# datavizweb/async-rl-tensorflow

Hardware: AMD Instinct MI355X
Metric: env-steps/sec (whole node), Pong-v0 84×84×4, 1/2/4/8 MI355X + CPU ref (higher is better)
Workload: dtype fp32; 1 GPU; Pong-v0, 256 envs batched per MI355X, n-step=5, A3C conv net (nips trunk); frames=M1: raw RGB 210x160x3 + screen, game=Pong-v0, trunk=nips, head=feed-forward, env=device, envs_per_gpu=256, n_step=5, action_size=6, algo=a3c, parallelism=dp1, hipgraph=False

## Files before the change

async-rl-tensorflow_amd/csrc/net_fwd.hip:

```cpp
#include <cstdlib>
#include "net.h"
#include "lstm.h"
#include "gemm.h"
#include "net_bwd.h"
#include "env_dev.h"
#include "screen_atari.h"
#include "net_head.h"

#define XB_BYTES (HIST * PLANE * 2)
#ifdef C2_FP32
#define L1S_BYTES (C1_P * L1S_LD * 4)
#else
#define L1T_LD 56
#define L1S_BYTES (C1_P * L1T_LD * 2)
#endif
#define CONV12_SMEM (XB_BYTES + L1S_BYTES)
#define CONV12_SMEM_U8 (HIST * PLANE + L1S_BYTES)

__device__ inline void split3_bits(float w, uint32_t& h, uint32_t& m, uint32_t& l) {
#pragma clang fp contract(off)
  h = bf16_rn_bits(w);
  const float r1 = w - __uint_as_float(h << 16);
  m = bf16_rn_bits(r1);
  const float r2 = r1 - __uint_as_float(m << 16);
// ... 233 lines not shown
      for (int t = 0; t < 3; ++t) bq[t] = bn[t];
    }
  }
#else
#pragma unroll
  for (int kh = 0; kh < C2_K; ++kh)
#pragma unroll
    for (int kw = 0; kw < C2_K; ++kw)
#pragma unroll
      for (int mi = 0; mi < 2; ++mi) {
        if (mi >= nm) break;
        f32x4 a = *(const f32x4*)(l1s + (pos0[mi] + kh * C1_O + kw) * L1S_LD + 4 * j4);
        f32x4& c = (kw & 1) ? acc2b[mi] : acc2[mi];
#pragma unroll
        for (int c4 = 0; c4 < 4; ++c4)
          c = __builtin_amdgcn_mfma_f32_16x16x4f32(a[c4], w2r[(kh * 4 + kw) * 4 + c4], c, 0, 0, 0);
      }
#endif
#pragma unroll
  for (int mi = 0; mi < 2; ++mi) acc2[mi] += acc2b[mi];
#pragma unroll
  for (int mi = 0; mi < 2; ++mi) {
    if (mi >= nm) break;
#pragma unroll
    for (int r = 0; r < 4; ++r) {
      const int q = 16 * (grp + 4 * mi) + 4 * j4 + r;
      const float v = fmaxf(acc2[mi][r] + bias2, 0.f);
      if (q < C2_Q) st_act(act_l2 + b * FLAT + q * C2_N + 16 * nt + i16, v);
      if (L2M && l2m) {
        const uint64_t bal = __ballot(v > 0.f);
        if (i16 == 0 && q < C2_Q)
          ((uint16_t*)l2m)[(b * C2_Q + q) * 2 + nt] = (uint16_t)(bal >> (16 * j4));
      }
    }
  }
}

static_assert(W1S_ELEMS * 2 <= L1S_BYTES, "conv1 weights staged in the l1 region");
template <bool SAVE_L1, bool EW, bool U8>
__device__ inline void conv12_core(const uint8_t* x8, const uint16_t* xb, float* l1s, int64_t b,
                                   const uint16_t* __restrict__ w1s, const float* __restrict__ b1,
                                   const float* __restrict__ W2, float* __restrict__ act_l1,
                                   float* __restrict__ act_l2, float (&w2r)[64], float bias2,
                                   uint64_t* dbg = nullptr, uint32_t* __restrict__ l2m = nullptr) {
  const int lane = threadIdx.x & 63;
  uint4* wl = (uint4*)l1s;
  for (int i = threadIdx.x; i < W1S_ELEMS / 8; i += blockDim.x) wl[i] = ((const uint4*)w1s)[i];
  __syncthreads();
  if (dbg && threadIdx.x == 0) dbg[11] = __builtin_readcyclecounter();
  f32x4 acc[C1_TILES];
#pragma unroll
  for (int i = 0; i < C1_TILES; ++i) acc[i] = (f32x4){0.f, 0.f, 0.f, 0.f};
  conv1_accum<U8, 0, HIST>(x8, xb, acc, [&](int f) { return __builtin_bit_cast(bf16x8, wl[f * 64 + lane]); });
  lds_only_barrier();
  conv12_finish<SAVE_L1, EW>(acc, l1s, b, w1s, b1, W2, act_l1, act_l2, w2r, bias2, dbg, l2m);
}


template <bool SAVE_L1, bool EW, bool U8>
__global__ void __launch_bounds__(512) k_conv12_fwd(StateAddr sa, int64_t B,
                                                    const uint16_t* __restrict__ w1s,
                                                    const float* __restrict__ b1,
                                                    const float* __restrict__ W2,
                                                    const float* __restrict__ b2,
                                                    float* __restrict__ act_l1,
                                                    float* __restrict__ act_l2,
                                                    uint32_t* __restrict__ l2m) {
  WGLOG(3);
  extern __shared__ __attribute__((aligned(16))) uint8_t smem[];
  uint16_t* xb = (uint16_t*)smem;
  uint8_t* x8 = smem;
  float* l1s = (float*)(smem + (U8 ? HIST * PLANE : XB_BYTES));
  const int64_t b = blockIdx.x;
  const int lane = threadIdx.x & 63, wid = threadIdx.x >> 6;
  const int i16 = lane & 15, j4 = lane >> 4;
  const int64_t tau0 = sa.tau_ptr ? *sa.tau_ptr : 0;
  WG_T0();

  constexpr int NCH = HIST * (PLANE / 16);
  constexpr int PER = (NCH + 511) / 512;
  auto stage_chunk = [&](int i, const uint4 v) {
    if constexpr (U8) {
      ((uint4*)x8)[i] = v;
      return;
    }
    const int c = i / (PLANE / 16), j = i - c * (PLANE / 16);
    const uint32_t w[4] = {v.x, v.y, v.z, v.w};
    uint32_t o[8];
#pragma unroll
    for (int q = 0; q < 4; ++q) {
      const float f0 = (float)(w[q] & 255u), f1 = (float)((w[q] >> 8) & 255u);
      const float f2 = (float)((w[q] >> 16) & 255u), f3 = (float)(w[q] >> 24);
      o[2 * q] = __builtin_amdgcn_perm(__float_as_uint(f1), __float_as_uint(f0), 0x07060302u);
      o[2 * q + 1] = __builtin_amdgcn_perm(__float_as_uint(f3), __float_as_uint(f2), 0x07060302u);
    }
    uint4* dst = (uint4*)(xb + c * PLANE + 16 * j);
    dst[0] = make_uint4(o[0], o[1], o[2], o[3]);
    dst[1] = make_uint4(o[4], o[5], o[6], o[7]);
  };
  auto chunk_src = [&](int i) -> uint4 {
    const int c = i / (PLANE / 16), j = i - c * (PLANE / 16);
    return ((const uint4*)state_plane(sa, b, c, tau0))[j];
  };
  uint4 sv[PER];
  if (EW) {
#pragma unroll
    for (int k = 0; k < PER; ++k) sv[k] = chunk_src(min((int)threadIdx.x + 512 * k, NCH - 1));
  } else {
    for (int i = threadIdx.x; i < NCH; i += 512) stage_chunk(i, chunk_src(i));
  }
  const int nt = wid & 1, grp = wid >> 1;
  float w2r[64];
#ifdef C2_FP32
  if (EW) {
#pragma unroll
    for (int kk = 0; kk < 16; ++kk)
#pragma unroll
      for (int c4 = 0; c4 < 4; ++c4) w2r[kk * 4 + c4] = W2[(kk * C1_N + 4 * j4 + c4) * C2_N + 16 * nt + i16];
  }
#endif
  const float bias2 = b2[16 * nt + i16];
  if (EW) {
#pragma unroll
    for (int k = 0; k < PER; ++k) {
      const int i = threadIdx.x + 512 * k;
      if (i < NCH) stage_chunk(i, sv[k]);
    }
  }

  conv12_core<SAVE_L1, EW, U8>(x8, xb, l1s, b, w1s, b1, W2, act_l1, act_l2, w2r, bias2, nullptr, l2m);
  WG_T1(act_l2 + b * FLAT);
}

template <int GAME = A3C_GAME_SYNTH>
__global__ void __launch_bounds__(256) k_head_fwd(const float* __restrict__ h3, int64_t B,
                                                  const float* __restrict__ Wp, const float* __restrict__ bp,
                                                  const float* __restrict__ Wv, const float* __restrict__ bv,
                                                  int A, int zs, float* __restrict__ z, HeadSelect sel) {
  WGLOG(4);
  __shared__ __attribute__((aligned(16))) f32x4 l3s[4][64];
  const int lane = threadIdx.x & 63;
  const int64_t b = (int64_t)blockIdx.x * 4 + (threadIdx.x >> 6);
  if (b >= B) return;
  float myz;
  if (sel.fc_part) {
    f32x4 fp[FC_NS];
#pragma unroll
    for (int w = 0; w < FC_NS; ++w) fp[w] = *(const f32x4*)(sel.fc_part + ((int64_t)w * B + b) * FC + 4 * lane);
    const f32x4 fb = *(const f32x4*)(sel.fc_bias + 4 * lane);
    f32x4 v = fp[0];
#pragma unroll
    for (int w = 1; w < FC_NS; ++w) v += fp[w];
#pragma unroll
    for (int c4 = 0; c4 < 4; ++c4) v[c4] = fmaxf(v[c4] + fb[c4], 0.f);
    l3s[threadIdx.x >> 6][lane] = v;
    if (sel.l3_out) *(f32x4*)(sel.l3_out + b * FC + 4 * lane) = v;
    myz = head_row((const float*)l3s[threadIdx.x >> 6], 0, Wp, bp, Wv, bv, A, lane);
  } else {
    myz = head_row(h3, b, Wp, bp, Wv, bv, A, lane);
  }
  if (lane < zs) z[b * zs + lane] = myz;
  if (sel.mode >= 0) (void)head_act<GAME>(myz, lane, A, sel, b);
  if (sel.adv_ptr && blockIdx.x == 0 && threadIdx.x == 0) *sel.adv_ptr += sel.adv_n;
}

template <int W = FC, bool PLAY = false, int GAME = A3C_GAME_SYNTH>
__device__ inline int32_t head_act_env(const float* __restrict__ h3, const float* __restrict__ Wp,
                                       const float* __restrict__ bp, const float* __restrict__ Wv,
                                       const float* __restrict__ bv, int A, int zs, float* __restrict__ z,
                                       const HeadSelect& sel, int64_t b, int64_t tau, uint64_t* dbg,
                                       const float* hrow = nullptr, const uint8_t* frozen = nullptr) {
  __shared__ int32_t s_act;
  __shared__ uint32_t s_draw, s_term;
  const int lane = threadIdx.x & 63, wid = threadIdx.x >> 6;
  const int e = (int)b;
  if constexpr (PLAY) {
    if (frozen[e]) return -1;
  }
  const int64_t nxt = ((tau + 1) & 1) * (int64_t)sel.par_E + e;
  if (wid == 0) {
    const float eps = sel_eps(sel, e, tau);
    u32x4 x;
    float myz;
    if constexpr (W == FC) {
      myz = hrow ? head_row(hrow, 0, Wp, bp, Wv, bv, A, lane, [&]() { x = action_draw(sel, b, tau); })
                 : head_row(h3, b, Wp, bp, Wv, bv, A, lane, [&]() { x = action_draw(sel, b, tau); });
    } else {
      auto mid = [&]() { x = action_draw(sel, b, tau); };
      myz = hrow ? head_row<decltype(mid), W>(hrow, 0, Wp, bp, Wv, bv, A, lane, mid)
                 : head_row<decltype(mid), W>(h3, b, Wp, bp, Wv, bv, A, lane, mid);
    }
    if (dbg) {
      if (lane == 0) dbg[1] = __builtin_readcyclecounter() + (uint64_t)(myz * 0.f);
    } else if (lane < zs) {
      z[b * zs + lane] = myz;
    }
    const int32_t a = select_with(myz, lane, A, sel.mode, x, eps);
    if (lane == 0) {
      sel.actions[b] = a;
      s_act = a;
      if (dbg) dbg[2] = __builtin_readcyclecounter() + (uint64_t)a * 0;
    }
  } else if (wid == 1 && lane == 0 && sel.env_on) {
    const int64_t cur = (tau & 1) * (int64_t)sel.par_E + e;
    const uint32_t id = (uint32_t)(sel.env_id_base + e);
    EnvState s = env_load(sel.envb, cur);
    uint32_t draw;
    if constexpr (GAME == A3C_GAME_CATCH) {
      draw = catch_act_pre(s, sel.envp.action_repeat);
    } else {
      draw = env_act_pre(s, sel.envp, id, !PLAY);
      if constexpr (!PLAY) sel.rewards[e] = fmaxf(-1.0f, fminf(1.0f, s.reward));
      if (sel.rewards_raw) sel.rewards_raw[e] = s.reward;
    }
    sel.terms[e] = (uint8_t)s.terminal;
    s_draw = draw;
    if constexpr (PLAY) {
      s_term = 0;
      env_store(sel.envb, nxt, s, false);
      env_store(sel.envb, cur, s, false);
    } else {
      s_term = s.terminal;
      if (s.terminal) {
        game_new_random_game<GAME>(s, sel.envp, id);
        env_store(sel.envb, nxt, s);
      } else {
        env_store(sel.envb, nxt, s, false);
      }
    }
    if (dbg) dbg[17] = __builtin_readcyclecounter();
  }
  __syncthreads();
  int32_t frame;
  if (sel.env_on) {
    float reward = 0.f;
    if constexpr (GAME == A3C_GAME_CATCH) {
      frame = catch_act_post(s_draw, (uint32_t)s_act, reward);
    } else {
      frame = env_frame_of(s_draw + sel.frame_salt, (uint32_t)s_act, sel.envp);
#ifdef A3C_ABL_FRAME
      frame = e & 63;
#endif
    }
    if (threadIdx.x == 0) {
      if constexpr (GAME == A3C_GAME_CATCH) {
        if constexpr (!PLAY) sel.rewards[e] = reward;
        if (sel.rewards_raw) sel.rewards_raw[e] = reward;
        if constexpr (PLAY) sel.envb.reward[nxt] = sel.envb.reward[(tau & 1) * (int64_t)sel.par_E + e] = reward;
      }
      sel.frames_out[e] = frame;
      if (!s_term) sel.envb.frame[nxt] = frame;
      if constexpr (PLAY) sel.envb.frame[(tau & 1) * (int64_t)sel.par_E + e] = frame;
    }
  } else {
    frame = sel.frames_out[b];
  }
  if (dbg && threadIdx.x == 0) dbg[3] = __builtin_readcyclecounter();
  return frame;
}

template <int HS_THREADS, int W = FC, int GAME = A3C_GAME_SYNTH>
__global__ void __launch_bounds__(HS_THREADS) k_head_screen(const float* __restrict__ h3,
                                                            const float* __restrict__ Wp,
                                                            const float* __restrict__ bp,
                                                            const float* __restrict__ Wv,
                                                            const float* __restrict__ bv, int A, int zs,
                                                            float* __restrict__ z, HeadSelect sel) {
  extern __shared__ __attribute__((aligned(16))) uint8_t smem[];
  const int64_t b = blockIdx.x;
  const int64_t tau = *sel.tau_ptr + sel.tau_add;
  WG_T0();
  uint64_t* dbg = nullptr;
#ifdef HS_TIMES
  dbg = blockIdx.x == HS_TIMES ? (uint64_t*)z : nullptr;
  if (dbg && threadIdx.x == 0) dbg[0] = __builtin_readcyclecounter();
#endif
  const int32_t frame = head_act_env<W, false, GAME>(h3, Wp, bp, Wv, bv, A, zs, z, sel, b, tau, dbg);
  uint8_t* slot = sel.ring + b * sel.R * PLANE + ((tau + 1) % sel.R) * PLANE;
  if (sel.frame84)
    atari::copy_frame84<HS_THREADS>(sel.pool + (int64_t)frame * PLANE, slot);
  else
    atari::screen_frame<HS_THREADS>(sel.pool + (int64_t)frame * (atari::IH * atari::IW * 3), slot, smem, dbg);
  WG_T1(z + b * zs);
}

template <int HS_THREADS, int W, int GAME = A3C_GAME_SYNTH>
__global__ void __launch_bounds__(HS_THREADS) k_head_screen_play(const float* __restrict__ h3,
                                                                 const float* __restrict__ Wp,
                                                                 const float* __restrict__ bp,
                                                                 const float* __restrict__ Wv,
                                                                 const float* __restrict__ bv, int A, int zs,
                                                                 float* __restrict__ z, HeadSelect sel,
                                                                 const uint8_t* __restrict__ frozen) {
  extern __shared__ __attribute__((aligned(16))) uint8_t smem[];
  const int64_t b = blockIdx.x;
  const int64_t tau = *sel.tau_ptr + sel.tau_add;
  const int32_t frame = head_act_env<W, true, GAME>(h3, Wp, bp, Wv, bv, A, zs, z, sel, b, tau, nullptr, nullptr, frozen);
  if (frame < 0) return;
  uint8_t* slot = sel.ring + b * sel.R * PLANE + ((tau + 1) % sel.R) * PLANE;
  if (sel.frame84)
    atari::copy_frame84<HS_THREADS>(sel.pool + (int64_t)frame * PLANE, slot);
  else
    atari::screen_frame<HS_THREADS>(sel.pool + (int64_t)frame * (atari::IH * atari::IW * 3), slot, smem, nullptr);
}

#define HSC_X8_OFF (((SCREEN_FRAME_SMEM_NOKV) + 15) / 16 * 16)
#define HSC_X8_BYTES ((HIST - 1) * 2 * 3 * 64 * 16)
#define HSC_SMEM (HSC_X8_OFF + HSC_X8_BYTES)
#define HSC_KV_OFF (PLANE * 2)
static_assert(L1S_BYTES <= SCREEN_FRAME_SMEM_NOKV, "l1 overlays the screen scratch");
static_assert(HSC_KV_OFF % 16 == 0 && HSC_KV_OFF + SCREEN_KV_BYTES <= HSC_X8_BYTES, "tap table in the x8 region");
static_assert(HSC_SMEM + 16 + 4096 <= 160 * 1024 - 82944, "rollout workgroup beside a compact conv backward one");
template <bool SAVE_L1, bool L2M, int GAME = A3C_GAME_SYNTH>
__global__ void __launch_bounds__(512) __attribute__((amdgpu_waves_per_eu(4))) k_head_screen_conv12(const float* __restrict__ h3,
                                                            const float* __restrict__ Wp,
                                                            const float* __restrict__ bp,
                                                            const float* __restrict__ Wv,
                                                            const float* __restrict__ bv, int A, int zs,
                                                            float* __restrict__ z, HeadSelect sel,
                                                            Conv12Next nx) {
  WGLOG(1);
  extern __shared__ __attribute__((aligned(16))) uint8_t smem[];
  uint8_t* x8 = smem + HSC_X8_OFF;
  const int64_t b = blockIdx.x;
  const int64_t tau = *sel.tau_ptr + sel.tau_add;
  const int64_t tau0 = *nx.sa.tau_ptr;
  WG_T0();
  unsigned long long* srec = span_rec(nx.sa, tau0);
  span_begin(srec);
  uint64_t* dbg = nullptr;
#ifdef HS_TIMES
  dbg = blockIdx.x == HS_TIMES ? (uint64_t*)z : nullptr;
  if (dbg && threadIdx.x == 0) dbg[0] = __builtin_readcyclecounter();
#endif
  constexpr int NCH3 = (HIST - 1) * (PLANE / 16);
  constexpr int PT = 512 - 128;
  constexpr int PER3 = (NCH3 + PT - 1) / PT;
  constexpr int NWF = (HIST - 1) * 2 * 3 * 64;
  constexpr int PERW = NWF / PT;
  static_assert(NWF % PT == 0 && NWF * 16 <= HSC_X8_BYTES, "old-plane conv1 weights in the x8 region");
  static_assert((HIST - 1) * PLANE * 2 <= 51 * 1024, "old planes as bf16 in the screen scratch");
  static_assert(PLANE * 2 <= HSC_X8_BYTES, "new plane as bf16 in the x8 region");
  const int fwid = threadIdx.x >> 6, flane = threadIdx.x & 63;
  const bool fold = sel.fc_part != nullptr;
  f32x4 fbias = {0.f, 0.f, 0.f, 0.f};
  f32x4 fpart[FC_NS];
  if (fold && fwid == 0) {
#pragma unroll
    for (int w = 0; w < FC_NS; ++w)
      fpart[w] = *(const f32x4*)(sel.fc_part + ((int64_t)w * gridDim.x + b) * FC + 4 * flane);
    fbias = *(const f32x4*)(sel.fc_bias + 4 * flane);
  }
  const int pt = (int)threadIdx.x - 128;
  uint4 pv[PER3];
  if (pt >= 0) {
#pragma unroll
    for (int k = 0; k < PER3; ++k) {
      const int i = min(pt + PT * k, NCH3 - 1);
      const int c = i / (PLANE / 16), j = i - c * (PLANE / 16);
      pv[k] = ((const uint4*)state_plane(nx.sa, b, c, tau0))[j];
    }
    const int wbase = (fwid - 2) * 64;
#pragma unroll
    for (int k = 0; k < PERW; ++k)
      glds16((const uint4*)nx.w1s + wbase + PT * k + flane, (uint4*)x8 + wbase + PT * k);
#ifdef HS_TIMES
    if (dbg && pt == 0) dbg[16] = __builtin_readcyclecounter() + (pv[0].x & 0);
#endif
  }
  const float* hrow = nullptr;
  if (fold) {
    f32x4* fl = (f32x4*)smem;
    if (fwid == 0) {
      f32x4 v = fpart[0];
#pragma unroll
      for (int w = 1; w < FC_NS; ++w) v += fpart[w];
#pragma unroll
      for (int c4 = 0; c4 < 4; ++c4) v[c4] = fmaxf(v[c4] + fbias[c4], 0.f);
      fl[flane] = v;
      *(f32x4*)(sel.l3_out + b * FC + 4 * flane) = v;
    }
    hrow = (const float*)fl;
  }
  const int32_t frame = head_act_env<FC, false, GAME>(h3, Wp, bp, Wv, bv, A, zs, z, sel, b, tau, dbg, hrow);
  uint16_t* xold = (uint16_t*)smem;
  uint4* wlds = (uint4*)x8;
  if (pt >= 0) {
    asm volatile("s_waitcnt vmcnt(0)" ::: "memory");
#pragma unroll
    for (int k = 0; k < PER3; ++k) {
      const int i = pt + PT * k;
      if (i < NCH3) {
        uint4* d = (uint4*)(xold + 16 * i);
        const uint2 a0 = atari::u8x4_to_bf16x4(pv[k].x), a1 = atari::u8x4_to_bf16x4(pv[k].y);
        const uint2 a2 = atari::u8x4_to_bf16x4(pv[k].z), a3 = atari::u8x4_to_bf16x4(pv[k].w);
        d[0] = make_uint4(a0.x, a0.y, a1.x, a1.y);
        d[1] = make_uint4(a2.x, a2.y, a3.x, a3.y);
      }
    }
  }
  const int lane = threadIdx.x & 63, wid = threadIdx.x >> 6;
  f32x4 acc[C1_TILES];
#pragma unroll
  for (int i = 0; i < C1_TILES; ++i) acc[i] = (f32x4){0.f, 0.f, 0.f, 0.f};
  auto conv1_old = [&]() {
    lds_only_barrier();
    conv1_accum<false, 0, HIST - 1, false>(nullptr, xold, acc,
                                           [&](int f) { return __builtin_bit_cast(bf16x8, wlds[f * 64 + lane]); });
    lds_only_barrier();
  };
  uint16_t* xnew = (uint16_t*)x8;
  uint8_t* slot = sel.ring + b * sel.R * PLANE + ((tau + 1) % sel.R) * PLANE;
  if (sel.frame84)
    atari::copy_frame84<512>(sel.pool + (int64_t)frame * PLANE, slot, xnew, conv1_old);
  else
    atari::screen_frame<512>(sel.pool + (int64_t)frame * (atari::IH * atari::IW * 3), slot, smem, dbg, xnew,
                             conv1_old, (int*)(x8 + HSC_KV_OFF));
  if (dbg && threadIdx.x == 0) dbg[9] = __builtin_readcyclecounter();
  uint4 wn[6];
#pragma unroll
  for (int f = 0; f < 6; ++f) wn[f] = ((const uint4*)nx.w1s)[((HIST - 1) * 6 + f) * 64 + lane];
  float w2r[64];
  const float bias2 = nx.b2[16 * (wid & 1) + (lane & 15)];
  __syncthreads();
  if (dbg && threadIdx.x == 0) dbg[11] = __builtin_readcyclecounter();
  conv1_accum<false, HIST - 1, HIST>(nullptr, xnew - (HIST - 1) * PLANE, acc, [&](int f) {
    return __builtin_bit_cast(bf16x8, wn[f - (HIST - 1) * 6]);
  });
  conv12_finish<SAVE_L1, false, L2M>(acc, (float*)smem, b, nx.w1s, nx.b1, nx.W2, SAVE_L1 ? nx.act_l1 : nullptr,
                                nx.act_l2, w2r, bias2, dbg, nx.l2m);
  span_end(srec);
  if (dbg) {
    __syncthreads();
    if (threadIdx.x == 0) dbg[10] = __builtin_readcyclecounter();
  }
  WG_T1(z + b * zs);
}

__global__ void __launch_bounds__(256) k_select(const float* __restrict__ z, int64_t B, int zs, int A,
                                                HeadSelect sel) {
  const int lane = threadIdx.x & 63;
  const int64_t b = (int64_t)blockIdx.x * 4 + (threadIdx.x >> 6);
  if (b >= B) return;
  float myz = lane < zs ? z[b * zs + lane] : 0.f;
  int32_t a = select_from_lanes(myz, lane, A, sel, b);
  if (lane == 0) sel.actions[b] = a;
}

int a3c_fc_fwd_launch(const float* A, const float* W, const float* bias, float* C, int64_t M, hipStream_t s,
                      const float* Wrows = nullptr);

template <int HS_THREADS, int W, int GAME = A3C_GAME_SYNTH>
__global__ void __launch_bounds__(HS_THREADS) k_head_screen_fold(const float* __restrict__ part, int nsplit,
                                                                 int64_t pstride, const float* __restrict__ fbias,
                                                                 float* __restrict__ hout,
                                                                 const float* __restrict__ Wp,
                                                                 const float* __restrict__ bp,
                                                                 const float* __restrict__ Wv,
                                                                 const float* __restrict__ bv, int A, int zs,
                                                                 float* __restrict__ z, HeadSelect sel) {
  extern __shared__ __attribute__((aligned(16))) uint8_t smem[];
  __shared__ __attribute__((aligned(16))) float hrow[W];
  const int64_t b = blockIdx.x;
  const int64_t tau = *sel.tau_ptr + sel.tau_add;
  for (int i = threadIdx.x; i < W; i += HS_THREADS) {
    const float v = fmaxf(sum_strided(part + b * W + i, nsplit, pstride) + fbias[i], 0.f);
    hrow[i] = v;
    hout[b * W + i] = v;
  }
  __syncthreads();
  const int32_t frame = head_act_env<W, false, GAME>(nullptr, Wp, bp, Wv, bv, A, zs, z, sel, b, tau, nullptr, hrow);
  uint8_t* slot = sel.ring + b * sel.R * PLANE + ((tau + 1) % sel.R) * PLANE;
  if (sel.frame84)
    atari::copy_frame84<HS_THREADS>(sel.pool + (int64_t)frame * PLANE, slot);
  else
    atari::screen_frame<HS_THREADS>(sel.pool + (int64_t)frame * (atari::IH * atari::IW * 3), slot, smem, nullptr);
}

static bool catch_on(const HeadSelect& sel) { return sel.env_on && sel.envp.game == A3C_GAME_CATCH; }
static int catch_fold_launch(const float* part, int nsplit, const float* fbias, float* l4, const float* Wp,
                             const float* bp, const float* Wv, const float* bv, int A, int zs, int64_t B, float* z,
                             const HeadSelect& sel, int nt, hipStream_t s);
static int catch_head_screen_launch(int W, const float* h, const float* Wp, const float* bp, const float* Wv,
                                    const float* bv, int A, int zs, int64_t B, float* z, const HeadSelect& sel, int nt,
                                    hipStream_t s);
static int catch_play_launch(int W, const float* h, const float* Wp, const float* bp, const float* Wv, const float* bv,
                             int A, int zs, int64_t B, float* z, const HeadSelect& sel, const uint8_t* frozen, int nt,
                             hipStream_t s);
static int catch_conv12_launch(const float* h, const float* Wp, const float* bp, const float* Wv, const float* bv, int A,
                               int zs, int64_t B, float* z, const HeadSelect& sel, const Conv12Next& nx, hipStream_t s);
static int catch_head_fwd_launch(const float* h, const float* Wp, const float* bp, const float* Wv, const float* bv, int A,
                                 int zs, int64_t B, float* z, const HeadSelect& sel, hipStream_t s);
static void catch_set_smem();

int a3c_head_screen_fold_launch(const float* part, int nsplit, const float* fbias, float* l4, const float* Wp,
                                const float* bp, const float* Wv, const float* bv, int A, int zs, int64_t B, float* z,
                                const HeadSelect& sel, hipStream_t s) {
  static const int env_t = (int)A3C_AB_KNOB("A3C_HS_THREADS", 0);
  const int nt = env_t ? env_t : (a3c_shared_gpu() ? 512 : 1024);
  const int64_t ps = B * 512;
  if (catch_on(sel)) return catch_fold_launch(part, nsplit, fbias, l4, Wp, bp, Wv, bv, A, zs, B, z, sel, nt, s);
  if (nt == 1024)
    hipLaunchKernelGGL((k_head_screen_fold<1024, 512>), dim3((unsigned)B), dim3(1024), SCREEN_FRAME_SMEM, s, part,
                       nsplit, ps, fbias, l4, Wp, bp, Wv, bv, A, zs, z, sel);
  else
    hipLaunchKernelGGL((k_head_screen_fold<512, 512>), dim3((unsigned)B), dim3(512), SCREEN_FRAME_SMEM, s, part,
                       nsplit, ps, fbias, l4, Wp, bp, Wv, bv, A, zs, z, sel);
  A3C_CHECK(hipGetLastError());
  return 0;
}

int a3c_head_screen_wide_launch(const float* l4, const float* Wp, const float* bp, const float* Wv, const float* bv,
                                int A, int zs, int64_t B, float* z, const HeadSelect& sel, hipStream_t s) {
  static const int env_t = (int)A3C_AB_KNOB("A3C_HS_THREADS", 0);
  const int nt = env_t ? env_t : (a3c_shared_gpu() ? 512 : 1024);
  if (catch_on(sel)) return catch_head_screen_launch(512, l4, Wp, bp, Wv, bv, A, zs, B, z, sel, nt, s);
  if (nt == 1024)
    hipLaunchKernelGGL((k_head_screen<1024, 512>), dim3((unsigned)B), dim3(1024), SCREEN_FRAME_SMEM, s, l4, Wp, bp,
                       Wv, bv, A, zs, z, sel);
  else
    hipLaunchKernelGGL((k_head_screen<512, 512>), dim3((unsigned)B), dim3(512), SCREEN_FRAME_SMEM, s, l4, Wp, bp, Wv,
                       bv, A, zs, z, sel);
  A3C_CHECK(hipGetLastError());
  return 0;
}

int a3c_head_screen_play_launch(int W, const float* h, const float* Wp, const float* bp, const float* Wv,
                                const float* bv, int A, int zs, int64_t B, float* z, const HeadSelect& sel,
                                const uint8_t* frozen, hipStream_t s) {
  if (B <= 0) return 0;
  if (!frozen || !sel.tau_ptr || !sel.env_on || !sel.ring || !sel.pool || !sel.rewards_raw || !sel.terms ||
      !sel.frames_out || !sel.actions || sel.mode < 0 || sel.par_E < B || (W != FC && W != 512))
    return a3c_set_error(A3C_ERR_INVALID, "a3c_head_screen_play", "bad argument");
  const int nt = a3c_shared_gpu() ? 512 : 1024;
  if (catch_on(sel)) return catch_play_launch(W, h, Wp, bp, Wv, bv, A, zs, B, z, sel, frozen, nt, s);
#define HSP_GO(T, WW) hipLaunchKernelGGL((k_head_screen_play<T, WW>), dim3((unsigned)B), dim3(T), SCREEN_FRAME_SMEM, s, h, \
                                         Wp, bp, Wv, bv, A, zs, z, sel, frozen)
  if (W == FC) {
    if (nt == 1024) HSP_GO(1024, FC);
    else HSP_GO(512, FC);
  } else {
    if (nt == 1024) HSP_GO(1024, 512);
    else HSP_GO(512, 512);
  }
#undef HSP_GO
  A3C_CHECK(hipGetLastError());
  return 0;
}

int a3c_head_screen_conv12_launch(const NetLayout& L, const float* P, const float* act_l3, int64_t B, float* z,
                                  const HeadSelect& sel, const Conv12Next& nx, hipStream_t s);
int a3c_forward_launch(const NetLayout& L, const float* params, const uint8_t* prep, const StateAddr& sa,
                       int64_t B, float* act_l1, float* act_l2, float* act_l3, float* z, const HeadSelect& sel,
                       hipStream_t s, const LstmStep* ls, bool skip_conv12, const Conv12Next* next,
                       float* fc_part, uint32_t* l2m, const uint8_t* play_frozen) {
  if (B <= 0) return 0;
  if (play_frozen && (next || fc_part || skip_conv12 || sel.mode < 0 || !sel.env_on || !sel.ring))
    return a3c_set_error(A3C_ERR_INVALID, "a3c_forward", "the play step runs unfused, with the device env and the fused screen");
  if (L.lstm != (ls != nullptr))
    return a3c_set_error(A3C_ERR_INVALID, "a3c_forward", "the LSTM head needs its recurrent state");
  const float* P = params;
  if (!skip_conv12) {
    int rc0 = a3c_conv12_launch(L, P, prep, sa, B, act_l1, act_l2, s, l2m);
    if (rc0) return rc0;
  }
  const bool part_lstm = fc_part && ls != nullptr;
  const bool part = fc_part && (part_lstm || (next ? sel.mode >= 0 && sel.env_on && sel.ring : sel.mode < 0));
  const bool fold_fc = part_lstm && ls->fc_tick;
  int rc = fold_fc ? a3c_fc_part_fold_launch(act_l2, (const float*)(prep + PREP_W1S_BYTES), fc_part, B, ls->fc_tick,
                                             P + L.off[T_FCB], act_l3, s)
         : part ? a3c_fc_part_launch(act_l2, (const float*)(prep + PREP_W1S_BYTES), fc_part, B, s)
                : a3c_fc_fwd_launch(act_l2, (const float*)(prep + PREP_W1S_BYTES), P + L.off[T_FCB], act_l3, B, s,
                                    P + L.off[T_FCW]);
  if (rc) return rc;
  const float* head_in = act_l3;
  if (ls) {
    LstmStep st = *ls;
    if (part_lstm && !fold_fc) {
      st.fc_part = fc_part;
      st.fc_bias = P + L.off[T_FCB];
      st.l3_out = act_l3;
    }
    rc = a3c_lstm_fwd_launch(P + L.off[T_LB], act_l3, st, B, s);
    if (rc) return rc;
    head_in = ls->h;
  }
  const float* Wv = L.algo == A3C_ALGO_A3C ? P + L.off[T_VW] : nullptr;
  const float* bv = L.algo == A3C_ALGO_A3C ? P + L.off[T_VB] : nullptr;
  if (sel.mode >= 0 && sel.env_on && sel.ring && next) {
    HeadSelect hs = sel;
    if (part && !part_lstm) {
      hs.fc_part = fc_part;
      hs.fc_bias = P + L.off[T_FCB];
      hs.l3_out = act_l3;
    }
    return a3c_head_screen_conv12_launch(L, P, head_in, B, z, hs, *next, s);
  }
  if (next) return a3c_set_error(A3C_ERR_INVALID, "a3c_forward", "conv fusion needs the fused env screen");
  if (play_frozen)
    return a3c_head_screen_play_launch(FC, head_in, P + L.off[T_HW], P + L.off[T_HB], Wv, bv, L.A, L.zs, B, z, sel,
                                       play_frozen, s);
  if (sel.mode >= 0 && sel.env_on && sel.ring)
    return a3c_head_screen_launch(L, P, head_in, B, z, sel, s);
  else {
    HeadSelect hs = sel;
    if (part && !part_lstm) {
      hs.fc_part = fc_part;
      hs.fc_bias = P + L.off[T_FCB];
      hs.l3_out = act_l3;
    }
    if (hs.mode >= 0 && catch_on(hs))
      return catch_head_fwd_launch(head_in, P + L.off[T_HW], P + L.off[T_HB], Wv, bv, L.A, L.zs, B, z, hs, s);
    hipLaunchKernelGGL(k_head_fwd<>, dim3((unsigned)((B + 3) / 4)), dim3(256), 0, s, head_in, B,
                       P + L.off[T_HW], P + L.off[T_HB], Wv, bv, L.A, L.zs, z, hs);
  }
  A3C_CHECK(hipGetLastError());
  return 0;
}

int a3c_head_screen_launch(const NetLayout& L, const float* P, const float* act_l3, int64_t B, float* z,
                           const HeadSelect& sel, hipStream_t s) {
  const float* Wv = L.algo == A3C_ALGO_A3C ? P + L.off[T_VW] : nullptr;
  const float* bv = L.algo == A3C_ALGO_A3C ? P + L.off[T_VB] : nullptr;
  static const int env_t = (int)A3C_AB_KNOB("A3C_HS_THREADS", 0);
  const int nt = env_t ? env_t : (a3c_shared_gpu() ? 512 : 1024);
  if (catch_on(sel))
    return catch_head_screen_launch(FC, act_l3, P + L.off[T_HW], P + L.off[T_HB], Wv, bv, L.A, L.zs, B, z, sel, nt, s);
  if (nt == 1024)
    hipLaunchKernelGGL(k_head_screen<1024>, dim3((unsigned)B), dim3(1024), SCREEN_FRAME_SMEM, s, act_l3,
                       P + L.off[T_HW], P + L.off[T_HB], Wv, bv, L.A, L.zs, z, sel);
  else
    hipLaunchKernelGGL(k_head_screen<512>, dim3((unsigned)B), dim3(512), SCREEN_FRAME_SMEM, s, act_l3,
                       P + L.off[T_HW], P + L.off[T_HB], Wv, bv, L.A, L.zs, z, sel);
  A3C_CHECK(hipGetLastError());
  return 0;
}

int a3c_head_screen_conv12_launch(const NetLayout& L, const float* P, const float* act_l3, int64_t B, float* z,
                                  const HeadSelect& sel, const Conv12Next& nx, hipStream_t s) {
  const float* Wv = L.algo == A3C_ALGO_A3C ? P + L.off[T_VW] : nullptr;
  const float* bv = L.algo == A3C_ALGO_A3C ? P + L.off[T_VB] : nullptr;
  if (!nx.sa.tau_ptr || !sel.tau_ptr)
    return a3c_set_error(A3C_ERR_INVALID, "a3c_head_screen_conv12", "device tau counters required");
  if (catch_on(sel))
    return catch_conv12_launch(act_l3, P + L.off[T_HW], P + L.off[T_HB], Wv, bv, L.A, L.zs, B, z, sel, nx, s);
#define HSC_GO(S, M) hipLaunchKernelGGL((k_head_screen_conv12<S, M>), dim3((unsigned)B), dim3(512), HSC_SMEM, s, act_l3, \
                                        P + L.off[T_HW], P + L.off[T_HB], Wv, bv, L.A, L.zs, z, sel, nx)
  if (nx.act_l1 && nx.l2m) HSC_GO(true, true);
  else if (nx.act_l1) HSC_GO(true, false);
  else if (nx.l2m) HSC_GO(false, true);
  else HSC_GO(false, false);
#undef HSC_GO
  A3C_CHECK(hipGetLastError());
  return 0;
}

int a3c_conv12_launch(const NetLayout& L, const float* P, const uint8_t* prep, const StateAddr& sa, int64_t B,
                      float* act_l1, float* act_l2, hipStream_t s, uint32_t* l2m) {
  if (!prep) return a3c_set_error(A3C_ERR_INVALID, "a3c_conv12_launch", "prepared forward weights missing");
  const uint16_t* w1s = (const uint16_t*)prep;
  const bool ew = !a3c_shared_gpu();
  static const int env_u8 = (int)A3C_AB_KNOB("A3C_C12_U8", -1);
  const bool u8 = env_u8 >= 0 ? env_u8 != 0 : !ew;
#define CONV12_ARGS sa, B, w1s, P + L.off[T_L1B], P + L.off[T_L2W], P + L.off[T_L2B], act_l1, act_l2, l2m
#define CONV12_GO(S, E, U) \
  hipLaunchKernelGGL((k_conv12_fwd<S, E, U>), dim3((unsigned)B), dim3(512), U ? CONV12_SMEM_U8 : CONV12_SMEM, s, CONV12_ARGS)
  if (u8) {
    if (act_l1 && ew) CONV12_GO(true, true, true);
    else if (act_l1) CONV12_GO(true, false, true);
    else if (ew) CONV12_GO(false, true, true);
    else CONV12_GO(false, false, true);
  } else {
    if (act_l1 && ew) CONV12_GO(true, true, false);
    else if (act_l1) CONV12_GO(true, false, false);
    else if (ew) CONV12_GO(false, true, false);
    else CONV12_GO(false, false, false);
  }
#undef CONV12_GO
#undef CONV12_ARGS
  A3C_CHECK(hipGetLastError());
  return 0;
}

int a3c_select_launch(const float* z, int64_t B, int zs, int A, const HeadSelect& sel, hipStream_t s) {
  if (B <= 0) return 0;
  hipLaunchKernelGGL(k_select, dim3((unsigned)((B + 3) / 4)), dim3(256), 0, s, z, B, zs, A, sel);
  A3C_CHECK(hipGetLastError());
  return 0;
}

void a3c_conv12_set_smem() {
#define C12_SMEM(S, E, U)                                                                        \
  (void)hipFuncSetAttribute((const void*)k_conv12_fwd<S, E, U>, hipFuncAttributeMaxDynamicSharedMemorySize, \
                            U ? CONV12_SMEM_U8 : CONV12_SMEM)
  C12_SMEM(true, true, false); C12_SMEM(true, false, false); C12_SMEM(false, true, false); C12_SMEM(false, false, false);
  C12_SMEM(true, true, true); C12_SMEM(true, false, true); C12_SMEM(false, true, true); C12_SMEM(false, false, true);
#undef C12_SMEM
  (void)hipFuncSetAttribute((const void*)k_head_screen_conv12<true, true>, hipFuncAttributeMaxDynamicSharedMemorySize,
                            HSC_SMEM);
  (void)hipFuncSetAttribute((const void*)k_head_screen_conv12<true, false>, hipFuncAttributeMaxDynamicSharedMemorySize,
                            HSC_SMEM);
  (void)hipFuncSetAttribute((const void*)k_head_screen_conv12<false, true>, hipFuncAttributeMaxDynamicSharedMemorySize,
                            HSC_SMEM);
  (void)hipFuncSetAttribute((const void*)k_head_screen_conv12<false, false>, hipFuncAttributeMaxDynamicSharedMemorySize,
                            HSC_SMEM);
  (void)hipFuncSetAttribute((const void*)k_head_screen<512>, hipFuncAttributeMaxDynamicSharedMemorySize,
                            SCREEN_FRAME_SMEM);
  (void)hipFuncSetAttribute((const void*)k_head_screen<1024>, hipFuncAttributeMaxDynamicSharedMemorySize,
                            SCREEN_FRAME_SMEM);
  (void)hipFuncSetAttribute((const void*)k_head_screen<512, 512>, hipFuncAttributeMaxDynamicSharedMemorySize,
                            SCREEN_FRAME_SMEM);
  (void)hipFuncSetAttribute((const void*)k_head_screen<1024, 512>, hipFuncAttributeMaxDynamicSharedMemorySize,
                            SCREEN_FRAME_SMEM);
  (void)hipFuncSetAttribute((const void*)k_head_screen_fold<512, 512>, hipFuncAttributeMaxDynamicSharedMemorySize,
                            SCREEN_FRAME_SMEM);
  (void)hipFuncSetAttribute((const void*)k_head_screen_fold<1024, 512>, hipFuncAttributeMaxDynamicSharedMemorySize,
                            SCREEN_FRAME_SMEM);
  (void)hipFuncSetAttribute((const void*)k_head_screen_play<512, FC>, hipFuncAttributeMaxDynamicSharedMemorySize,
                            SCREEN_FRAME_SMEM);
  (void)hipFuncSetAttribute((const void*)k_head_screen_play<1024, FC>, hipFuncAttributeMaxDynamicSharedMemorySize,
                            SCREEN_FRAME_SMEM);
  (void)hipFuncSetAttribute((const void*)k_head_screen_play<512, 512>, hipFuncAttributeMaxDynamicSharedMemorySize,
                            SCREEN_FRAME_SMEM);
  (void)hipFuncSetAttribute((const void*)k_head_screen_play<1024, 512>, hipFuncAttributeMaxDynamicSharedMemorySize,
                            SCREEN_FRAME_SMEM);
  catch_set_smem();
}

template <int NW>
__global__ void __launch_bounds__(64 * NW) k_fc_fwd(const float* __restrict__ A, const float* __restrict__ Wp,
                                                    const float* __restrict__ bias, float* __restrict__ C, int M,
                                                    int xcd_rows) {
  __shared__ f32x4 red[NW - 1][64];
  const int lane = threadIdx.x & 63, wid = threadIdx.x >> 6;
  const int i16 = lane & 15, j4 = lane >> 4;
  int ct = blockIdx.x, mt = blockIdx.y;
  int m0, rstride = 1;
// ... 497 lines not shown
```

Before: 4.904 million env-steps/s.

## Compute old-plane conv1 directly from global in idle waves and hand off accumulators

```diff
diff --git a/async-rl-tensorflow_amd/csrc/net_fwd.hip b/async-rl-tensorflow_amd/csrc/net_fwd.hip
--- a/async-rl-tensorflow_amd/csrc/net_fwd.hip
+++ b/async-rl-tensorflow_amd/csrc/net_fwd.hip
@@ -559,6 +559,79 @@
     atari::copy_frame84<HS_THREADS>(sel.pool + (int64_t)frame * PLANE, slot);
   else
     atari::screen_frame<HS_THREADS>(sel.pool + (int64_t)frame * (atari::IH * atari::IW * 3), slot, smem, nullptr);
+}
+
+#define C1O_TILES 5
+#define C1O_HAND_TILES 7
+#define C1O_HAND_BYTES (C1O_HAND_TILES * 64 * 16)
+#ifndef C1O_DEPTH
+#define C1O_DEPTH 1
+#endif
+__device__ inline int conv1_hand_slot(int m) { return (m & 7) ? 4 + (m >> 3) : (m >> 3); }
+__device__ inline void conv1_old_direct(const StateAddr& sa, int64_t b, int64_t tau0,
+                                        const uint16_t* __restrict__ w1s, f32x4 (&acc)[C1_TILES], f32x4* hand) {
+  const int lane = threadIdx.x & 63, wid = __builtin_amdgcn_readfirstlane(threadIdx.x >> 6);
+  const int i16 = lane & 15, j4 = lane >> 4;
+  const int k = wid - 2;
+  const int nt = wid == 7 ? 5 : 4;
+  int m[C1O_TILES];
+#pragma unroll
+  for (int i = 0; i < 3; ++i) m[i] = wid + 8 * i;
+  m[3] = k < 4 ? 8 * k : 1 + 8 * (k - 4);
+  m[4] = 17;
+  int off[C1O_TILES];
+#pragma unroll
+  for (int i = 0; i < C1O_TILES; ++i) {
+    const int p = min(16 * m[i] + i16, C1_P - 1);
+    const int oy = p / C1_O, ox = p - oy * C1_O;
+    off[i] = (C1_S * oy + j4) * IMG + C1_S * ox;
+  }
+  const uint8_t* pl[HIST - 1];
+#pragma unroll
+  for (int c = 0; c < HIST - 1; ++c) pl[c] = state_plane(sa, b, c, tau0);
+  constexpr int NS = (HIST - 1) * 2;
+  uint4 w[NS][3];
+  uint32_t q[NS][C1O_TILES][2];
+  auto read_step = [&](int st) {
+    const int c = st >> 1, h2 = st & 1;
+#pragma unroll
+    for (int t = 0; t < 3; ++t) w[st][t] = ((const uint4*)w1s)[((2 * c + h2) * 3 + t) * 64 + lane];
+#pragma unroll
+    for (int i = 0; i < C1O_TILES; ++i) {
+      if (i >= nt) break;
+      const uint32_t* p = (const uint32_t*)(pl[c] + off[i] + 4 * h2 * IMG);
+      q[st][i][0] = p[0];
+      q[st][i][1] = p[1];
+    }
+  };
+  f32x4 a5[C1O_TILES];
+#pragma unroll
+  for (int i = 0; i < C1O_TILES; ++i) a5[i] = (f32x4){0.f, 0.f, 0.f, 0.f};
+#pragma unroll
+  for (int st = 0; st < C1O_DEPTH && st < NS; ++st) read_step(st);
+#pragma unroll
+  for (int st = 0; st < NS; ++st) {
+    if (st + C1O_DEPTH < NS) read_step(st + C1O_DEPTH);
+    bf16x8 a[C1O_TILES];
+#pragma unroll
+    for (int i = 0; i < C1O_TILES; ++i) {
+      if (i >= nt) break;
+      a[i] = u8x8_to_bf16(q[st][i][0], q[st][i][1]);
+    }
+#pragma unroll
+    for (int t = 0; t < 3; ++t) {
+      const bf16x8 wt = __builtin_bit_cast(bf16x8, w[st][t]);
+#pragma unroll
+      for (int i = 0; i < C1O_TILES; ++i) {
+        if (i >= nt) break;
+        a5[i] = __builtin_amdgcn_mfma_f32_16x16x32_bf16(a[i], wt, a5[i], 0, 0, 0);
+      }
+    }
+  }
+#pragma unroll
+  for (int i = 0; i < 3; ++i) acc[i] = a5[i];
+  hand[conv1_hand_slot(m[3]) * 64 + lane] = a5[3];
+  if (nt == 5) hand[conv1_hand_slot(m[4]) * 64 + lane] = a5[4];
 }
 
 #define HSC_X8_OFF (((SCREEN_FRAME_SMEM_NOKV) + 15) / 16 * 16)
@@ -590,6 +663,23 @@
   dbg = blockIdx.x == HS_TIMES ? (uint64_t*)z : nullptr;
   if (dbg && threadIdx.x == 0) dbg[0] = __builtin_readcyclecounter();
 #endif
+#ifdef HS_TIMES
+  uint64_t t_c1old = 0;
+#endif
+  static_assert(PLANE * 2 <= HSC_X8_BYTES, "new plane as bf16 in the x8 region");
+  f32x4 acc[C1_TILES];
+#pragma unroll
+  for (int i = 0; i < C1_TILES; ++i) acc[i] = (f32x4){0.f, 0.f, 0.f, 0.f};
+#ifndef HSC_STAGED_CONV1
+  static_assert(C1O_HAND_BYTES <= HSC_KV_OFF, "accumulator hand-over below the tap table in the x8 region");
+  f32x4* hand = (f32x4*)x8;
+  if ((int)(threadIdx.x >> 6) >= 2) {
+    conv1_old_direct(nx.sa, b, tau0, nx.w1s, acc, hand);
+#ifdef HS_TIMES
+    t_c1old = __builtin_readcyclecounter() + (uint64_t)(acc[0][0] * 0.f);
+#endif
+  }
+#else
   constexpr int NCH3 = (HIST - 1) * (PLANE / 16);
   constexpr int PT = 512 - 128;
   constexpr int PER3 = (NCH3 + PT - 1) / PT;
@@ -597,7 +687,7 @@
   constexpr int PERW = NWF / PT;
   static_assert(NWF % PT == 0 && NWF * 16 <= HSC_X8_BYTES, "old-plane conv1 weights in the x8 region");
   static_assert((HIST - 1) * PLANE * 2 <= 51 * 1024, "old planes as bf16 in the screen scratch");
-  static_assert(PLANE * 2 <= HSC_X8_BYTES, "new plane as bf16 in the x8 region");
+#endif
   const int fwid = threadIdx.x >> 6, flane = threadIdx.x & 63;
   const bool fold = sel.fc_part != nullptr;
   f32x4 fbias = {0.f, 0.f, 0.f, 0.f};
@@ -608,6 +698,7 @@
       fpart[w] = *(const f32x4*)(sel.fc_part + ((int64_t)w * gridDim.x + b) * FC + 4 * flane);
     fbias = *(const f32x4*)(sel.fc_bias + 4 * flane);
   }
+#ifdef HSC_STAGED_CONV1
   const int pt = (int)threadIdx.x - 128;
   uint4 pv[PER3];
   if (pt >= 0) {
@@ -625,6 +716,7 @@
     if (dbg && pt == 0) dbg[16] = __builtin_readcyclecounter() + (pv[0].x & 0);
 #endif
   }
+#endif
   const float* hrow = nullptr;
   if (fold) {
     f32x4* fl = (f32x4*)smem;
@@ -640,6 +732,20 @@
     hrow = (const float*)fl;
   }
   const int32_t frame = head_act_env<FC, false, GAME>(h3, Wp, bp, Wv, bv, A, zs, z, sel, b, tau, dbg, hrow);
+  const int lane = threadIdx.x & 63, wid = threadIdx.x >> 6;
+#ifndef HSC_STAGED_CONV1
+  auto acc_reload = [&]() {
+    if (wid < 2) {
+#pragma unroll
+      for (int i = 0; i < C1_TILES; ++i)
+        if (i < conv1_ntiles(wid)) acc[i] = hand[(4 * wid + i) * 64 + lane];
+    }
+  };
+  auto acc_reload84 = [&]() {
+    acc_reload();
+    lds_only_barrier();
+  };
+#else
   uint16_t* xold = (uint16_t*)smem;
   uint4* wlds = (uint4*)x8;
   if (pt >= 0) {
@@ -656,23 +762,22 @@
       }
     }
   }
-  const int lane = threadIdx.x & 63, wid = threadIdx.x >> 6;
-  f32x4 acc[C1_TILES];
-#pragma unroll
-  for (int i = 0; i < C1_TILES; ++i) acc[i] = (f32x4){0.f, 0.f, 0.f, 0.f};
   auto conv1_old = [&]() {
     lds_only_barrier();
     conv1_accum<false, 0, HIST - 1, false>(nullptr, xold, acc,
                                            [&](int f) { return __builtin_bit_cast(bf16x8, wlds[f * 64 + lane]); });
     lds_only_barrier();
   };
+  auto& acc_reload = conv1_old;
+  auto& acc_reload84 = conv1_old;
+#endif
   uint16_t* xnew = (uint16_t*)x8;
   uint8_t* slot = sel.ring + b * sel.R * PLANE + ((tau + 1) % sel.R) * PLANE;
   if (sel.frame84)
-    atari::copy_frame84<512>(sel.pool + (int64_t)frame * PLANE, slot, xnew, conv1_old);
+    atari::copy_frame84<512>(sel.pool + (int64_t)frame * PLANE, slot, xnew, acc_reload84);
   else
     atari::screen_frame<512>(sel.pool + (int64_t)frame * (atari::IH * atari::IW * 3), slot, smem, dbg, xnew,
-                             conv1_old, (int*)(x8 + HSC_KV_OFF));
+                             acc_reload, (int*)(x8 + HSC_KV_OFF));
   if (dbg && threadIdx.x == 0) dbg[9] = __builtin_readcyclecounter();
   uint4 wn[6];
 #pragma unroll
@@ -690,6 +795,10 @@
   if (dbg) {
     __syncthreads();
     if (threadIdx.x == 0) dbg[10] = __builtin_readcyclecounter();
+#ifdef HS_TIMES
+    if (lane == 0 && wid == 2 && t_c1old) dbg[16] = t_c1old;
+    if (lane == 0 && wid == 7 && t_c1old) dbg[18] = t_c1old;
+#endif
   }
   WG_T1(z + b * zs);
 }
```

Result: no change. 4.952 million env-steps/s, median of 6 (+1.0%).
